# JunyiPeng00/wespeaker_hubert

Hardware: AMD Instinct MI355X
Metric: embeddings/sec on 5s 16kHz utts (higher is better)
Workload: dtype f32 (bf16x3 split MFMA, fp32 accumulate)

## Files before the change

### wespeaker_hubert_amd/csrc/conv_gemm.hip

```cpp
#include "gemm_common.h"

namespace wsp {

namespace {

constexpr int BK = 32;
constexpr int LDK = BK + 4;

template <int WM, int WN, int TM, int TN, int AMODE, bool UNI>
__global__ __launch_bounds__(256, 2) void conv_gemm_f32(const ConvGemmArgs p) {
  constexpr int BM = WM * TM * 32;
  constexpr int BN = WN * TN * 32;
  constexpr int AR = BM / 32;
  constexpr int BR = BN / 32;
  static_assert(WM * WN == 4, "4 waves");

  extern __shared__ __attribute__((aligned(16))) float smem[];
  float* As = smem;
  float* Bs = smem + 2 * BM * LDK;

  const int tid = threadIdx.x;
  const int lane = tid & 63;
  const int wave = tid >> 6;
  const int ntiles = p.N / BN;
// ... 89 lines not shown

template <int WM, int WN, int TM, int TN>
void launch_tile(const ConvGemmArgs& p, hipStream_t s) {
  const bool uni = uniform_ktiles(p);
  if (p.amode == kAAdd) {
    if (uni) launch_k<WM, WN, TM, TN, kAAdd, true>(p, s);
    else launch_k<WM, WN, TM, TN, kAAdd, false>(p, s);
  } else {
    if (uni) launch_k<WM, WN, TM, TN, kACat, true>(p, s);
    else launch_k<WM, WN, TM, TN, kACat, false>(p, s);
  }
}

}

int conv_gemm_tile_for(int N) { return (N % 128 == 0) ? 0 : 1; }

void launch_conv_gemm(const ConvGemmArgs& args, hipStream_t s) {
  const ConvGemmArgs p = normalized(args);
  check_conv_args(p, "conv_gemm");
  WSP_CHECK(!p.colsum, "conv_gemm: column sums are a bf16x3-kernel epilogue");
  WSP_CHECK(!p.conv2d && p.N % 64 == 0, "conv_gemm (f32): 1-D convs with N % 64 == 0 only");
  WSP_CHECK(!p.gcols || p.gcols % 64 == 0, "conv_gemm (f32): grouped columns must be a multiple of 64");
  WSP_CHECK(!p.sc2d && !p.lnmode && !p.gate,
            "conv_gemm (f32): conv3 + shortcut, the LayerNorm fold and the gated A tail run on tile family 7");
  if (conv_gemm_tile_for(p.N) == 0 && !p.gcols)
    launch_tile<2, 2, 2, 2>(p, s);
  else
    launch_tile<4, 1, 1, 2>(p, s);
}

}
```

### wespeaker_hubert_amd/csrc/conv_gemm_x3.hip

```cpp
#include "conv_gemm_x3_impl.h"

namespace wsp {

int conv_gemm_x3_block_rows(const ConvGemmArgs& p, int variant) {
  if (p.N % 64 != 0 || (p.gcols && p.gcols % 64 != 0)) return 128;
  if (p.gcols || p.N % 128 != 0) return 128;
  return variant == 3 ? 128 : 256;
}

namespace {
__global__ __launch_bounds__(256) void colsum_mean_kernel(const double* __restrict__ part, int bm, int T, int N,
                                                          float* __restrict__ out, int ldo) {
  const int b = blockIdx.y;
  const int n = blockIdx.x * 256 + threadIdx.x;
  if (n >= N) return;
  const long r0 = (long)b * T, r1 = r0 + T;
  double v = 0.0;
  for (long mt = r0 / bm; mt * bm < r1; ++mt) {
    const int slot = (mt * bm) / T == b ? 0 : 1;
    v += part[((size_t)mt * 2 + slot) * N + n];
  }
  out[(long)b * ldo + n] = (float)(v / (double)T);
}
}

void launch_colsum_mean(const double* part, int block_rows, int T, int B, int N, float* out, int ldo,
                        hipStream_t s) {
  WSP_CHECK(block_rows > 0 && T >= block_rows && B > 0 && N > 0, "colsum_mean: bad shape");
  hipLaunchKernelGGL(colsum_mean_kernel, dim3((N + 255) / 256, B), dim3(256), 0, s, part, block_rows, T, N, out,
                     ldo);
  WSP_HIP(hipGetLastError());
}

bool conv_gemm_x3_gate_ok(const ConvGemmArgs& args, int variant) {
  return variant == 7 && args.gate && x3::g256_gate_supported(normalized(args));
}

void launch_conv_gemm_x3(const ConvGemmArgs& args, const void* whi, const void* wlo, int variant,
                         hipStream_t s) {
  const ConvGemmArgs p = normalized(args);
  check_conv_args(p, "conv_gemm_x3");
  if (p.colsum) {
    const int bm = conv_gemm_x3_block_rows(p, variant);
    WSP_CHECK(!p.seg && !p.row_bias && !p.conv2d && p.T >= bm,
              "conv_gemm_x3: column sums need a uniform batch with T >= block rows and no row bias");
  }
  WSP_CHECK(p.Kp % 64 == 0, "conv_gemm_x3: packed K must be a multiple of 64");
  WSP_CHECK(variant >= 3 && variant <= 7, "conv_gemm_x3: tile family must be 3, 4, 5, 6 or 7");
  const __bf16* h = static_cast<const __bf16*>(whi);
  const __bf16* l = static_cast<const __bf16*>(wlo);
  x3::TileFn f;
  WSP_CHECK(!p.lnmode || (variant == 7 && x3::g256_supported(p)),
            "conv_gemm_x3: the LayerNorm fold runs on tile family 7 only");
  WSP_CHECK(!p.sc2d || (variant == 7 && x3::g256_supported(p)),
            "conv_gemm_x3: conv3 + shortcut runs on tile family 7 only (N % 256 == 0, 16-B aligned operands)");
  WSP_CHECK(!p.gate || (variant == 7 && x3::g256_gate_supported(p)),
            "conv_gemm_x3: the gated A tail runs on tile family 7 only (conv_gemm_x3_gate_ok)");
  if (variant == 7 && x3::g256_supported(p)) {
    x3::t_g256(p, h, l, s);
    return;
  }
  if (variant == 7) variant = 6;
  if (p.N % 64 != 0 || (p.gcols && p.gcols % 64 != 0)) {
    f = x3::t_4x1_1x1;
  } else if (p.gcols) {
    f = variant >= 5 ? x3::t_8x1_1x2_sw : x3::t_4x1_1x2;
  } else if (p.N % 128 != 0) {
    f = x3::t_4x1_1x2;
  } else if (variant == 3) {
    f = x3::t_2x2_2x2_sw;
  } else if (variant == 4) {
    f = x3::t_4x2_2x2_sw;
  } else if (p.N % 256 == 0) {
    f = variant == 6 ? x3::t_4x2_2x4_mf16 : x3::t_4x2_2x4_sw1;
// ... 8 lines not shown
```

### wespeaker_hubert_amd/csrc/conv_gemm_x3_impl.h

```cpp
#pragma once

#include <type_traits>

#include "gemm_common.h"

namespace wsp {

namespace {

typedef __bf16 bf16x8 __attribute__((ext_vector_type(8)));
typedef __bf16 bf16x4 __attribute__((ext_vector_type(4)));

constexpr int BK = 32;

template <bool SWZ, int MF = 32>
struct Lds {
  static constexpr int ROWB = SWZ ? 64 : 80;
  static constexpr int SKEW = SWZ ? 0 : 64;
  __device__ __forceinline__ static int off(int row, int byte) {
    static_assert(MF == 32 || SWZ, "16x16 fragments need the swizzled rows");
    if constexpr (SWZ && MF == 16)
      return row * 64 + ((((byte >> 4) ^ (0x1320 >> (4 * ((row >> 2) & 3)))) & 3) << 4) + (byte & 15);
    else if constexpr (SWZ) return row * 64 + ((((byte >> 4) ^ (row >> 2)) & 3) << 4) + (byte & 15);
    else return row * 80 + byte;
// ... 281 lines not shown
    if (p.res && p.role == 2)
      launch_x3_k<WM, WN, TM, TN, kACat, true, 2, false, SWZ, NSET>(p, whi, wlo, s);
    else
      launch_x3_k<WM, WN, TM, TN, kACat, true, 0, false, SWZ, NSET>(p, whi, wlo, s);
  } else {
    launch_x3_k<WM, WN, TM, TN, kACat, true, 0, false, SWZ, NSET, MF>(p, whi, wlo, s);
  }
}

}

namespace x3 {
using TileFn = void (*)(const ConvGemmArgs&, const __bf16*, const __bf16*, hipStream_t);
void t_4x1_1x1(const ConvGemmArgs&, const __bf16*, const __bf16*, hipStream_t);
void t_4x1_1x2(const ConvGemmArgs&, const __bf16*, const __bf16*, hipStream_t);
void t_8x1_1x2_sw(const ConvGemmArgs&, const __bf16*, const __bf16*, hipStream_t);
void t_2x2_2x2_sw(const ConvGemmArgs&, const __bf16*, const __bf16*, hipStream_t);
void t_4x2_2x2_sw(const ConvGemmArgs&, const __bf16*, const __bf16*, hipStream_t);
void t_4x2_2x4_sw1(const ConvGemmArgs&, const __bf16*, const __bf16*, hipStream_t);
void t_4x2_2x4_mf16(const ConvGemmArgs&, const __bf16*, const __bf16*, hipStream_t);
bool g256_supported(const ConvGemmArgs&);
bool g256_gate_supported(const ConvGemmArgs&);
void t_g256(const ConvGemmArgs&, const __bf16*, const __bf16*, hipStream_t);
}

}
```

### wespeaker_hubert_amd/csrc/conv_gemm_x3_t6.hip

```cpp
#include "conv_gemm_x3_impl.h"

namespace wsp {
namespace {

typedef __attribute__((address_space(3))) void lds_void;
constexpr int kGA = 256 * 128, kGW = 256 * 64, kGStage = kGA + 2 * kGW;

__device__ __forceinline__ int g_aslot(int r, int c) { return r * 128 + ((c ^ ((r >> 1) & 5)) << 4); }

__device__ __forceinline__ void g_dma(__amdgpu_buffer_rsrc_t r, unsigned char* lds, int voff) {
  __builtin_amdgcn_raw_ptr_buffer_load_lds(r, (lds_void*)lds, 16, voff, 0, 0, 0);
}

constexpr int kGEpiLd = 132;
constexpr int kGEpiBytes = 8 * 32 * kGEpiLd * 4;
typedef unsigned u32x4 __attribute__((ext_vector_type(4)));

constexpr int kLnMaxParts = 8;
__device__ __forceinline__ void g_ln_row(const ConvGemmArgs& p, int row, float& mu, float& rstd) {
  const float* s = p.ln_in + (size_t)row * p.ln_parts * 2;
  float m = s[0], m2 = s[1];
#pragma unroll
  for (int k = 1; k < kLnMaxParts; ++k) {
    if (k < p.ln_parts) {
      const float d = s[2 * k] - m;
      m += d * (1.f / (float)(k + 1));
      m2 += s[2 * k + 1] + d * d * (128.f * (float)k / (float)(k + 1));
    }
  }
  mu = m;
  rstd = 1.f / sqrtf(m2 / (128.f * (float)p.ln_parts) + p.ln_eps);
}

template <int R>
__device__ __forceinline__ void g_ln_pieces(float (&m)[R], float (&m2)[R]) {
  float n = 4.f;
  auto merge = [&](int i, float mo, float m2o) {
    const float d = mo - m[i];
    m[i] = 0.5f * (m[i] + mo);
    m2[i] = (m2[i] + m2o) + d * d * (0.5f * n);
  };
#define WSP_DPP(v, ctrl) __builtin_bit_cast(float, __builtin_amdgcn_mov_dpp(__builtin_bit_cast(int, v), ctrl, 0xF, 0xF, false))
#pragma unroll
  for (int i = 0; i < R; ++i) merge(i, WSP_DPP(m[i], 0xB1), WSP_DPP(m2[i], 0xB1));
  n *= 2.f;
#pragma unroll
  for (int i = 0; i < R; ++i) merge(i, WSP_DPP(m[i], 0x4E), WSP_DPP(m2[i], 0x4E));
  n *= 2.f;
#pragma unroll
  for (int i = 0; i < R; ++i) merge(i, WSP_DPP(m[i], 0x141), WSP_DPP(m2[i], 0x141));
  n *= 2.f;
#pragma unroll
  for (int i = 0; i < R; ++i) merge(i, WSP_DPP(m[i], 0x140), WSP_DPP(m2[i], 0x140));
  n *= 2.f;
#undef WSP_DPP
#define WSP_BC15(v) \
  __builtin_bit_cast(float, __builtin_amdgcn_update_dpp(0, __builtin_bit_cast(int, v), 0x142, 0xA, 0xF, false))
#pragma unroll
  for (int i = 0; i < R; ++i) merge(i, WSP_BC15(m[i]), WSP_BC15(m2[i]));
#undef WSP_BC15
}

template <int ACT, bool RB, bool RES, int LNM = 0>
__device__ __forceinline__ void g_epilogue_rows(const ConvGemmArgs& p, f32x4 (&acc)[4][8], int m0, int n0, int wm,
                                                int wn, int wave, int lane, unsigned char* smem, float lmu = 0.f,
                                                float lrs = 1.f) {
  float* stg = reinterpret_cast<float*>(smem) + wave * 32 * kGEpiLd;
  const int c16 = lane & 15, q = lane >> 4;
  const int cl = 4 * (lane & 31);
  const int col = n0 + wn * 128 + cl;
  const f32x4 bv = p.bias ? *reinterpret_cast<const f32x4*>(p.bias + col) : f32x4{0.f, 0.f, 0.f, 0.f};
  const f32x4 sc = p.scale ? *reinterpret_cast<const f32x4*>(p.scale + col) : f32x4{1.f, 1.f, 1.f, 1.f};
  const f32x4 sh = p.scale ? *reinterpret_cast<const f32x4*>(p.shift + col) : f32x4{0.f, 0.f, 0.f, 0.f};
  f32x4 lcs{0.f, 0.f, 0.f, 0.f}, lg{1.f, 1.f, 1.f, 1.f}, lb{0.f, 0.f, 0.f, 0.f};
  if constexpr ((LNM & 2) != 0) lcs = *reinterpret_cast<const f32x4*>(p.ln_cs + col);
  if constexpr ((LNM & 4) != 0) {
    lg = *reinterpret_cast<const f32x4*>(p.ln_g + col);
    lb = *reinterpret_cast<const f32x4*>(p.ln_b + col);
  }
  const int lparts = p.N / 128, lpart = (n0 + wn * 128) / 128;
  const __amdgpu_buffer_rsrc_t ro = make_rsrc(p.out);
  const __amdgpu_buffer_rsrc_t rres = make_rsrc(RES ? p.res : p.out);
#pragma unroll
  for (int h = 0; h < 2; ++h) {
    float pm[(LNM & 1) ? 16 : 1], pm2[(LNM & 1) ? 16 : 1];
#pragma unroll
    for (int i2 = 0; i2 < 2; ++i2)
#pragma unroll
      for (int j = 0; j < 8; ++j)
#pragma unroll
        for (int r = 0; r < 4; ++r) stg[(i2 * 16 + 4 * q + r) * kGEpiLd + j * 16 + c16] = acc[2 * h + i2][j][r];
    asm volatile("s_waitcnt lgkmcnt(0)" ::: "memory");
#pragma unroll
    for (int u = 0; u < 16; ++u) {
      const int rl = 2 * u + (lane >> 5);
      const int row = m0 + wm * 64 + h * 32 + rl;
      const bool ok = row < p.M;
      const f32x4 x = *reinterpret_cast<const f32x4*>(stg + rl * kGEpiLd + cl);
      f32x4 rv{0.f, 0.f, 0.f, 0.f}, rb{0.f, 0.f, 0.f, 0.f};
      if constexpr (RES) rv = bload4(rres, ok ? (row * p.ldres + col) * 4 : kOOB);
      if constexpr (RB) {
        const int rowc = ok ? row : p.M - 1;
        const int ub = p.seg ? seg_of(p.seg, p.nseg, rowc) : rowc / p.T;
        rb = *reinterpret_cast<const f32x4*>(p.row_bias + (size_t)ub * p.N + col);
      }
      float mu = 0.f, rstd = 1.f;
      if constexpr ((LNM & 6) != 0) {
        auto rd = [](float v, int l) {
          return __builtin_bit_cast(float, __builtin_amdgcn_readlane(__builtin_bit_cast(int, v), l));
        };
        mu = lane < 32 ? rd(lmu, h * 32 + 2 * u) : rd(lmu, h * 32 + 2 * u + 1);
        rstd = lane < 32 ? rd(lrs, h * 32 + 2 * u) : rd(lrs, h * 32 + 2 * u + 1);
      }
      f32x4 y;
#pragma unroll
      for (int e = 0; e < 4; ++e) {
        float v;
        if constexpr ((LNM & 2) != 0) v = (x[e] - mu * lcs[e]) * rstd + bv[e];
        else v = x[e] + bv[e];
        if constexpr ((LNM & 4) != 0) v += (rv[e] - mu) * rstd * lg[e] + lb[e];
        else if constexpr (RES) v += rv[e];
        if constexpr (RB) v += rb[e];
        if constexpr (ACT == kActRelu) v = fmaxf(v, 0.f);
        else if constexpr (ACT == kActTanh) v = tanhf(v);
        else if constexpr (ACT == kActGelu) v = gelu_as(v);
        y[e] = v * sc[e] + sh[e];
      }
      __builtin_amdgcn_raw_buffer_store_b128(__builtin_bit_cast(u32x4, y), ro, ok ? (row * p.ldo + col) * 4 : kOOB, 0,
                                             0);
      if constexpr ((LNM & 1) != 0) {
        pm[u] = ((y[0] + y[1]) + (y[2] + y[3])) * 0.25f;
        float q2 = 0.f;
#pragma unroll
        for (int e = 0; e < 4; ++e) q2 += (y[e] - pm[u]) * (y[e] - pm[u]);
        pm2[u] = q2;
      }
    }
    if constexpr ((LNM & 1) != 0) {
      g_ln_pieces<16>(pm, pm2);
      if ((lane & 31) == 16) {
#pragma unroll
        for (int u = 0; u < 16; ++u) {
          const int row = m0 + wm * 64 + h * 32 + 2 * u + (lane >> 5);
          if (row < p.M) *reinterpret_cast<float2*>(p.ln_out + ((size_t)row * lparts + lpart) * 2) = float2{pm[u], pm2[u]};
        }
      }
    }
    asm volatile("s_waitcnt lgkmcnt(0)" ::: "memory");
  }
}

constexpr int kGCsLd = 68;
constexpr int kGCsBytes = 8 * 64 * kGCsLd * 4;
template <int ACT>
__device__ __forceinline__ void g_epilogue_cs(const ConvGemmArgs& p, f32x4 (&acc)[4][8], int m0, int n0, int wm,
                                              int wn, int wave, int lane, unsigned char* smem) {
  float* stg = reinterpret_cast<float*>(smem) + wave * 64 * kGCsLd;
  const int c16 = lane & 15, q = lane >> 4;
  const int cl = 4 * c16;
  const __amdgpu_buffer_rsrc_t ro = make_rsrc(p.out);
  const int nb = min((m0 / p.T + 1) * p.T, p.M) - m0, mb = p.M - m0;
  unsigned side0 = 0, side1 = 0;
#pragma unroll
  for (int k = 0; k < 16; ++k) {
    const int rr = wm * 64 + (k >> 2) * 16 + 4 * q + (k & 3);
    side0 |= (rr < nb ? 1u : 0u) << k;
    side1 |= (rr >= nb && rr < mb ? 1u : 0u) << k;
  }
  double rs[8][2];
#pragma unroll
  for (int pp = 0; pp < 2; ++pp) {
#pragma unroll
    for (int i = 0; i < 4; ++i)
// ... 370 lines not shown
```

### wespeaker_hubert_amd/csrc/ecapa_model.cpp

```cpp
#include "astp_fused.h"
#include "model_impl.h"
#include "res2_chain.h"
#include "xi_pool.h"

namespace wsp {

namespace {
struct Ecapa final : Model::Impl {
  using Impl::Impl;
  int C = 512;
  bool glob = false;
  bool xi = false;
  ConvW layer1;
  struct Block {
    ConvW c1, c3, res2[7];
    LinW se1, se2;
    void* r2w = nullptr;
    float *r2b = nullptr, *r2s = nullptr, *r2t = nullptr;
  } blk[3];
  ConvW conv, pool1, pool2;
  ConvW conv_g;
  void* pool2_frag = nullptr;
  LinW pool1_ctx;
  float *prior_mean = nullptr, *prior_logprec = nullptr;
// ... 231 lines not shown
  ConvGemmArgs gcat{};
  gcat.amode = kACat;
  gcat.a[0] = x[2];
  gcat.a[1] = x[3];
  gcat.a[2] = x[4];
  gcat.cseg[1] = C;
  gcat.cseg[2] = 2 * C;
  gcat.cseg[3] = 3 * C;
  gcat.lda[0] = gcat.lda[1] = gcat.lda[2] = C;
  const ConvW& wcat = opt.cat_gate ? conv_g : conv;
  bool fold = false;
  if (opt.cat_gate && opt.gate_fold && opt.precision == 1) {
    ConvGemmArgs g = gcat;
    g.a[2] = h3;
    g.gate = W.gate;
    g.ldg = C;
    g.gate_k0 = 2 * C;
    fill(g, wcat, M, T, 1, 0, xp, 1536, kActRelu, nullptr, true, seg, B);
    fold = conv_gemm_x3_gate_ok(g, opt.x3_variant);
    if (fold) gcat = g;
  }

  gemm("layer1", layer1, feats, feat_dim, x[1], C, M, T, 1, 2, kActRelu, s, seg, B);
  for (int li = 0; li < 3; ++li) {
    const Block& b = blk[li];
    const int dil = li + 2;
    const float* xin = x[li + 1];
    gemm("conv1x1_CxC", b.c1, xin, C, h1, C, M, T, 1, 0, kActRelu, s, seg, B, nullptr, true, 1);
    if (opt.precision == 1 && opt.res2_fused && b.r2w) {
      Res2Args r{};
      r.x = h1;
      r.out = h2;
      r.ldx = r.ldo = C;
      r.M = M;
      r.T = T;
      r.dil = dil;
      r.variant = w == 128 ? opt.res2_variant : std::min(opt.res2_variant, 3);
      r.rout = res2_chain_rout(dil, r.variant, M);
      r.seg = seg;
      r.nseg = B;
      r.w = b.r2w;
      r.bias = b.r2b;
      r.scale = b.r2s;
      r.shift = b.r2t;
      run("res2_k3", 7 * 2.0 * M * w * 3 * w, s, [&] { launch_res2_chain(r, w, s); });
    } else {
      for (int i = 0; i < 7; ++i) {
        ConvGemmArgs g{};
        g.amode = i == 0 ? kACat : kAAdd;
        if (i == 0) {
          one_operand(g, h1, C, w);
// ... 4 lines not shown
        }
        gemm3("res2_k3", g, b.res2[i], dil, dil, h2 + i * w, C);
      }
    }
    {
      ConvGemmArgs g{};
      g.amode = kACat;
      g.a[0] = h2;
      g.a[1] = h1 + 7 * w;
      g.a[2] = h1;
      g.cseg[1] = 7 * w;
      g.cseg[2] = g.cseg[3] = C;
      g.role = 1;
      if (se_fused) g.colsum = W.sesum;
      gemm3("conv1x1_CxC", g, b.c3, 1, 0, h3, C);
    }
    run("se", 0, s, [&] {
      if (se_fused) launch_colsum_mean(W.sesum, se_bm, T, B, C, W.gmean, C, s);
      else launch_frame_stats(h3, C, B, T, C, W.gmean, C, 0, 0, s, seg);
      launch_small_linear({W.gmean, C, b.se1.wt, b.se1.bias, W.ghid, 128, B, C, 128, 1}, s);
      launch_small_linear({W.ghid, 128, b.se2.wt, b.se2.bias, W.gate, C, B, 128, C, 3}, s);
    });
    if (li == 2 && fold) continue;
    run("se.scale", 0, s, [&] {
      launch_residual_scale(opt.cat_gate && li == 2 ? nullptr : xin, h3, W.gate, x[li + 2], B, T, C, s, seg, M);
    });
  }
  gemm3("conv_cat", gcat, wcat, 1, 0, xp, 1536);
  if (glob) {
    run("glob_ctx", 0, s, [&] {
      launch_frame_stats(xp, 1536, B, T, 1536, W.gstats, 3072, 1, 1536, s, seg);
      launch_small_linear({W.gstats, 3072, pool1_ctx.wt, pool1_ctx.bias, W.rowb, 128, B, 3072, 128, 0}, s);
    });
  }
  if (xi) {
    gemm("xi_lin1", pool1, xp, 1536, W.att, 256, M, T, 1, 0, kActRelu, s, seg, B);
    gemm("xi_lin2", pool2, W.att, 256, W.logit, 1536, M, T, 1, 0, kActNone, s, seg, B);
    const XiPoolArgs a{W.logit, 1536, xp, 1536, prior_mean, prior_logprec, B, T, 1536, seg, W.pooled, 1536};
    run("xi_pool", 0, s, [&] { launch_xi_pool(a, s); });
    run("head", 0, s, [&] {
      launch_small_linear({W.pooled, 1536, head.wt, head.bias, embed, embed_dim, B, 1536, embed_dim, 0}, s);
    });
    return;
  }
  gemm("pool_linear1", pool1, xp, 1536, W.att, 128, M, T, 1, 0, kActTanh, s, seg, B, glob ? W.rowb : nullptr, !glob);
  if (opt.precision == 1 && opt.astp_fused) {
// ... 13 lines not shown
```

### wespeaker_hubert_amd/csrc/kernels.h

```cpp
#pragma once

#include <vector>

#include "common.h"

namespace wsp {

enum AMode { kACat = 0, kAAdd = 1 };
enum Act { kActNone = 0, kActRelu = 1, kActTanh = 2, kActGelu = 3 };

struct ConvGemmArgs {
  const float* a[3];
  int lda[3];
  int cseg[4];
  int cin, taps, dil, pad;
  int M, T, N;
  const float* w;
  int K, Kp;
  const float* bias;
  const float* row_bias;
  const float* res;
  int ldres;
  const float* scale;
  const float* shift;
  float* out;
  int ldo;
  int act;
  int amode;
  int role;
  int conv2d;
  int Fi, Ti, Fo, To, stride, kw;
  int sc2d;
  int gcols, gcin;
  const int* seg;
  const int* iseg;
  int nseg;
  double* colsum;
  int lnmode;
  float* ln_out;
  const float* ln_in;
  int ln_parts;
  const float* ln_cs;
  const float* ln_g;
  const float* ln_b;
  float ln_eps;
  const float* gate;
  int ldg, gate_k0;
};

inline ConvGemmArgs normalized(ConvGemmArgs p) {
  if (!p.conv2d && !p.sc2d) {
    if (p.stride <= 0) p.stride = 1;
    if (p.Ti <= 0) p.Ti = p.T;
  }
  return p;
}

int conv_gemm_x3_block_rows(const ConvGemmArgs& p, int variant);
void launch_colsum_mean(const double* part, int block_rows, int T, int B, int N, float* out, int ldo,
                        hipStream_t s);
void launch_conv_gemm_x3(const ConvGemmArgs& p, const void* whi, const void* wlo, int variant,
                         hipStream_t s);
bool conv_gemm_x3_gate_ok(const ConvGemmArgs& p, int variant);


void launch_conv_gemm(const ConvGemmArgs& p, hipStream_t s);
int conv_gemm_tile_for(int N);

struct SmallLinearArgs {
  const float* in;
  int ldin;
  const float* wt;
  const float* bias;
  float* out;
  int ldo;
  int R, K, N;
  int act;
  float* scratch = nullptr;
  size_t scratch_floats = 0;
};
void launch_small_linear(const SmallLinearArgs& p, hipStream_t s);
size_t small_linear_scratch_floats(int R, int N, int K);


void launch_frame_stats(const float* x, int ldx, int B, int T, int C, float* out, int ldo,
                        int with_std, int std_off, hipStream_t s, const int* seg = nullptr);
// ... 86 lines not shown
```

### wespeaker_hubert_amd/csrc/model.cpp

```cpp
#include "model_impl.h"

namespace wsp {

int detail::chunk_for(int B, size_t bytes) {
  const int bc = std::min((int)std::max<size_t>(1, kOperandCap / bytes), B);
  const int chunks = (B + bc - 1) / bc;
  return (B + chunks - 1) / chunks;
}

void Model::Impl::add(const std::string& n, std::vector<int64_t> shape) {
  idx[n] = (int)params.size();
  params.push_back(Param{n, std::move(shape), {}, false});
}
void Model::Impl::add_bn(const std::string& p, int64_t c) {
  add(p + ".weight", {c});
  add(p + ".bias", {c});
  add(p + ".running_mean", {c});
  add(p + ".running_var", {c});
  add(p + ".num_batches_tracked", {});
}
const std::vector<float>& Model::Impl::P(const std::string& n) const {
  auto it = idx.find(n);
  WSP_CHECK(it != idx.end(), "missing parameter " + n);
  const Param& p = params[it->second];
// ... 243 lines not shown
    }
  impl->prof = on;
}

namespace {
struct Opt {
  const char* key;
  int Options::*field;
  int lo, hi, hole;
  const char* err;
};
using I = Options;
constexpr int kNoHole = -1000;
const Opt kOpts[] = {
    {"precision", &I::precision, 0, 1, kNoHole, "precision must be 0 (f32) or 1 (bf16x3)"},
    {"streams", &I::streams, 1, 8, kNoHole, "streams must be 1..8"},
    {"layer", &I::layer, -1, 12, kNoHole, "layer must be -1 (weighted sum) or 0..12"},
    {"in_planes", &I::in_planes, 32, 64, kNoHole, "in_planes must be 32 or 64"},
    {"res2_fused", &I::res2_fused, 0, 1, kNoHole, "res2_fused must be 0 or 1"},
    {"cam_fused", &I::cam_fused, 0, 1, kNoHole, "cam_fused must be 0 (separate BN-ReLU pass) or 1 (GEMM prologue)"},
    {"ib_fused", &I::ib_fused, 0, 1, kNoHole, "ib_fused must be 0 (conv1, depthwise conv, conv3) or 1 (conv1, fused tail)"},
    {"cat_gate", &I::cat_gate, 0, 1, kNoHole, "cat_gate must be 0 or 1"},
    {"gate_fold", &I::gate_fold, 0, 1, kNoHole, "gate_fold must be 0 or 1"},
    {"res_prefetch", &I::res_prefetch, 0, 1, kNoHole, "res_prefetch must be 0 or 1"},
    {"res_tail", &I::res_tail, 0, 2, kNoHole, "res_tail must be 0 (off), 1 (tail + next conv1) or 2 (tail alone)"},
    {"sc_fuse", &I::sc_fuse, 0, 3, kNoHole, "sc_fuse must be 0 .. 3 (bit 0: one GEMM, bit 1: in the tail)"},
    {"c1_stage_fuse", &I::c1_stage_fuse, 0, 1, kNoHole, "c1_stage_fuse must be 0 or 1"},
    {"astp_fused", &I::astp_fused, 0, 3, kNoHole,
     "astp_fused must be 0 (linear2 GEMM + pooling kernel) or 1 (fused)"},
    {"attn_pipe", &I::attn_pipe, 0, 1, kNoHole, "attn_pipe must be 0 or 1"},
    {"pos_conv", &I::pos_conv, 0, 1, kNoHole,
     "pos_conv must be 0 (grouped implicit GEMM) or 1 (direct grouped conv)"},
    {"ln_fold", &I::ln_fold, 0, 1, kNoHole, "ln_fold must be 0 (LayerNorm kernels) or 1 (folded into the GEMMs)"},
    {"tail_batch", &I::tail_batch, 0, 1, kNoHole,
     "tail_batch must be 0 (CNN layers 4-6 per chunk) or 1 (batch-wide)"},
    {"res2_variant", &I::res2_variant, 0, 4, 1,
     "res2_variant must be 0 (4 waves, 2 x 2), 2 (4 waves on N, 4 W k-steps in flight), 3 (8 waves) "
     "or 4 (halo-free strips, c1024 widths; else as 3)"},
    {"x3_variant", &I::x3_variant, 0, 9, kNoHole,
     "x3_variant must be 3, 4, 5, 6 (5 on 16x16x32 MFMAs) or 7 (6 staged by LDS-DMA)"},
    {"conv3x3_img", &I::conv3x3_img, 0, 3, kNoHole,
     "conv3x3_img must be 0 (off), 1 (32 / 64 channels) or 2 / 3 (also 128)"},
};
const Opt& find_opt(const std::string& key) {
  for (const Opt& o : kOpts)
    if (key == o.key) return o;
// ... 52 lines not shown
```

### wespeaker_hubert_amd/csrc/model_impl.h

```cpp
#pragma once

#include <hip/hip_runtime.h>

#include <cmath>
#include <cstdint>
#include <algorithm>
#include <map>
#include <string>
#include <vector>

#include "kernels.h"
#include "model.h"
#include "pack.h"

namespace wsp {

namespace detail {

constexpr double kBnEps = 1e-5;

struct DevBuf {
  std::vector<void*> ptrs;
  ~DevBuf() {
    for (void* p : ptrs) (void)hipFree(p);
// ... 52 lines not shown
  std::vector<float> host;
  bool set = false;
  int64_t numel() const {
    int64_t n = 1;
    for (auto s : shape) n *= s;
    return n;
  }
};

struct ProfEntry {
  std::vector<std::pair<hipEvent_t, hipEvent_t>> ev;
  size_t used = 0;
  double flops = 0;
};

struct Options {
  int precision = 1;
  int x3_variant = 5;
  int streams = 1;
  int res2_fused = 1;
  int res2_variant = 4;
  int cat_gate = 1;
  int gate_fold = 1;
  int astp_fused = 1;
  int in_planes = 32;
  int conv3x3_img = 2;
  int res_prefetch = 1;
  int res_tail = 1;
  int sc_fuse = 3;
  int c1_stage_fuse = 1;
  int layer = -1;
  int attn_pipe = 1;
  int pos_conv = 1;
  int ln_fold = 0;
  int tail_batch = 1;
  int cam_fused = 1;
  int ib_fused = 0;
};

struct Model::Impl {
  std::string arch;
  int feat_dim = 80, embed_dim = 192;
  bool emb_bn = false, two_emb = false;
  Options opt;
  std::vector<Param> params;
  std::map<std::string, int> idx;
// ... 81 lines not shown
```

Measured before the change: 25730.

## Fuse SE residual scaling into next block's conv1x1 GEMM A-load (seam kernel)

Adds a seam GEMM kernel that builds the next block's conv1x1 input on the fly, as residual plus h3 times the SE gate, while loading A tiles. It writes the scaled residual out as a side product and feeds it into the bf16x3 MFMA GEMM. This removes the separate residual_scale kernel launch and one round trip of the activation through memory between ECAPA blocks. The cost is a new specialized kernel with extra A-side arithmetic and stores in its main loop, enabled by default when shape and alignment checks pass.

```diff
diff --git a/wespeaker_hubert_amd/csrc/conv_gemm.hip b/wespeaker_hubert_amd/csrc/conv_gemm.hip
--- a/wespeaker_hubert_amd/csrc/conv_gemm.hip
+++ b/wespeaker_hubert_amd/csrc/conv_gemm.hip
@@ -135,8 +135,8 @@
   WSP_CHECK(!p.colsum, "conv_gemm: column sums are a bf16x3-kernel epilogue");
   WSP_CHECK(!p.conv2d && p.N % 64 == 0, "conv_gemm (f32): 1-D convs with N % 64 == 0 only");
   WSP_CHECK(!p.gcols || p.gcols % 64 == 0, "conv_gemm (f32): grouped columns must be a multiple of 64");
-  WSP_CHECK(!p.sc2d && !p.lnmode && !p.gate,
-            "conv_gemm (f32): conv3 + shortcut, the LayerNorm fold and the gated A tail run on tile family 7");
+  WSP_CHECK(!p.sc2d && !p.lnmode && !p.gate && !p.seam_h && !p.seam_out,
+            "conv_gemm (f32): conv3 + shortcut, the LayerNorm fold, the gated A tail and the seam run on tile family 7");
   if (conv_gemm_tile_for(p.N) == 0 && !p.gcols)
     launch_tile<2, 2, 2, 2>(p, s);
   else
diff --git a/wespeaker_hubert_amd/csrc/conv_gemm_x3.hip b/wespeaker_hubert_amd/csrc/conv_gemm_x3.hip
--- a/wespeaker_hubert_amd/csrc/conv_gemm_x3.hip
+++ b/wespeaker_hubert_amd/csrc/conv_gemm_x3.hip
@@ -36,6 +36,10 @@
   return variant == 7 && args.gate && x3::g256_gate_supported(normalized(args));
 }
 
+bool conv_gemm_x3_seam_ok(const ConvGemmArgs& args, int variant) {
+  return variant == 7 && args.seam_h && x3::seam_supported(normalized(args));
+}
+
 void launch_conv_gemm_x3(const ConvGemmArgs& args, const void* whi, const void* wlo, int variant,
                          hipStream_t s) {
   const ConvGemmArgs p = normalized(args);
@@ -50,6 +54,12 @@
   const __bf16* h = static_cast<const __bf16*>(whi);
   const __bf16* l = static_cast<const __bf16*>(wlo);
   x3::TileFn f;
+  if (p.seam_h || p.seam_out) {
+    WSP_CHECK(variant == 7 && x3::seam_supported(p),
+              "conv_gemm_x3: the seam runs on tile family 7 only (conv_gemm_x3_seam_ok)");
+    x3::t_seam(p, h, l, s);
+    return;
+  }
   WSP_CHECK(!p.lnmode || (variant == 7 && x3::g256_supported(p)),
             "conv_gemm_x3: the LayerNorm fold runs on tile family 7 only");
   WSP_CHECK(!p.sc2d || (variant == 7 && x3::g256_supported(p)),
diff --git a/wespeaker_hubert_amd/csrc/conv_gemm_x3_g.h b/wespeaker_hubert_amd/csrc/conv_gemm_x3_g.h
--- /dev/null
+++ b/wespeaker_hubert_amd/csrc/conv_gemm_x3_g.h
@@ -0,0 +1,156 @@
+#pragma once
+
+#include "conv_gemm_x3_impl.h"
+
+namespace wsp {
+namespace {
+
+typedef __attribute__((address_space(3))) void lds_void;
+constexpr int kGA = 256 * 128, kGW = 256 * 64, kGStage = kGA + 2 * kGW;
+
+__device__ __forceinline__ int g_aslot(int r, int c) { return r * 128 + ((c ^ ((r >> 1) & 5)) << 4); }
+
+__device__ __forceinline__ void g_dma(__amdgpu_buffer_rsrc_t r, unsigned char* lds, int voff) {
+  __builtin_amdgcn_raw_ptr_buffer_load_lds(r, (lds_void*)lds, 16, voff, 0, 0, 0);
+}
+
+constexpr int kGEpiLd = 132;
+constexpr int kGEpiBytes = 8 * 32 * kGEpiLd * 4;
+typedef unsigned u32x4 __attribute__((ext_vector_type(4)));
+
+constexpr int kLnMaxParts = 8;
+__device__ __forceinline__ void g_ln_row(const ConvGemmArgs& p, int row, float& mu, float& rstd) {
+  const float* s = p.ln_in + (size_t)row * p.ln_parts * 2;
+  float m = s[0], m2 = s[1];
+#pragma unroll
+  for (int k = 1; k < kLnMaxParts; ++k) {
+    if (k < p.ln_parts) {
+      const float d = s[2 * k] - m;
+      m += d * (1.f / (float)(k + 1));
+      m2 += s[2 * k + 1] + d * d * (128.f * (float)k / (float)(k + 1));
+    }
+  }
+  mu = m;
+  rstd = 1.f / sqrtf(m2 / (128.f * (float)p.ln_parts) + p.ln_eps);
+}
+
+template <int R>
+__device__ __forceinline__ void g_ln_pieces(float (&m)[R], float (&m2)[R]) {
+  float n = 4.f;
+  auto merge = [&](int i, float mo, float m2o) {
+    const float d = mo - m[i];
+    m[i] = 0.5f * (m[i] + mo);
+    m2[i] = (m2[i] + m2o) + d * d * (0.5f * n);
+  };
+#define WSP_DPP(v, ctrl) __builtin_bit_cast(float, __builtin_amdgcn_mov_dpp(__builtin_bit_cast(int, v), ctrl, 0xF, 0xF, false))
+#pragma unroll
+  for (int i = 0; i < R; ++i) merge(i, WSP_DPP(m[i], 0xB1), WSP_DPP(m2[i], 0xB1));
+  n *= 2.f;
+#pragma unroll
+  for (int i = 0; i < R; ++i) merge(i, WSP_DPP(m[i], 0x4E), WSP_DPP(m2[i], 0x4E));
+  n *= 2.f;
+#pragma unroll
+  for (int i = 0; i < R; ++i) merge(i, WSP_DPP(m[i], 0x141), WSP_DPP(m2[i], 0x141));
+  n *= 2.f;
+#pragma unroll
+  for (int i = 0; i < R; ++i) merge(i, WSP_DPP(m[i], 0x140), WSP_DPP(m2[i], 0x140));
+  n *= 2.f;
+#undef WSP_DPP
+#define WSP_BC15(v) \
+  __builtin_bit_cast(float, __builtin_amdgcn_update_dpp(0, __builtin_bit_cast(int, v), 0x142, 0xA, 0xF, false))
+#pragma unroll
+  for (int i = 0; i < R; ++i) merge(i, WSP_BC15(m[i]), WSP_BC15(m2[i]));
+#undef WSP_BC15
+}
+
+template <int ACT, bool RB, bool RES, int LNM = 0>
+__device__ __forceinline__ void g_epilogue_rows(const ConvGemmArgs& p, f32x4 (&acc)[4][8], int m0, int n0, int wm,
+                                                int wn, int wave, int lane, unsigned char* smem, float lmu = 0.f,
+                                                float lrs = 1.f) {
+  float* stg = reinterpret_cast<float*>(smem) + wave * 32 * kGEpiLd;
+  const int c16 = lane & 15, q = lane >> 4;
+  const int cl = 4 * (lane & 31);
+  const int col = n0 + wn * 128 + cl;
+  const f32x4 bv = p.bias ? *reinterpret_cast<const f32x4*>(p.bias + col) : f32x4{0.f, 0.f, 0.f, 0.f};
+  const f32x4 sc = p.scale ? *reinterpret_cast<const f32x4*>(p.scale + col) : f32x4{1.f, 1.f, 1.f, 1.f};
+  const f32x4 sh = p.scale ? *reinterpret_cast<const f32x4*>(p.shift + col) : f32x4{0.f, 0.f, 0.f, 0.f};
+  f32x4 lcs{0.f, 0.f, 0.f, 0.f}, lg{1.f, 1.f, 1.f, 1.f}, lb{0.f, 0.f, 0.f, 0.f};
+  if constexpr ((LNM & 2) != 0) lcs = *reinterpret_cast<const f32x4*>(p.ln_cs + col);
+  if constexpr ((LNM & 4) != 0) {
+    lg = *reinterpret_cast<const f32x4*>(p.ln_g + col);
+    lb = *reinterpret_cast<const f32x4*>(p.ln_b + col);
+  }
+  const int lparts = p.N / 128, lpart = (n0 + wn * 128) / 128;
+  const __amdgpu_buffer_rsrc_t ro = make_rsrc(p.out);
+  const __amdgpu_buffer_rsrc_t rres = make_rsrc(RES ? p.res : p.out);
+#pragma unroll
+  for (int h = 0; h < 2; ++h) {
+    float pm[(LNM & 1) ? 16 : 1], pm2[(LNM & 1) ? 16 : 1];
+#pragma unroll
+    for (int i2 = 0; i2 < 2; ++i2)
+#pragma unroll
+      for (int j = 0; j < 8; ++j)
+#pragma unroll
+        for (int r = 0; r < 4; ++r) stg[(i2 * 16 + 4 * q + r) * kGEpiLd + j * 16 + c16] = acc[2 * h + i2][j][r];
+    asm volatile("s_waitcnt lgkmcnt(0)" ::: "memory");
+#pragma unroll
+    for (int u = 0; u < 16; ++u) {
+      const int rl = 2 * u + (lane >> 5);
+      const int row = m0 + wm * 64 + h * 32 + rl;
+      const bool ok = row < p.M;
+      const f32x4 x = *reinterpret_cast<const f32x4*>(stg + rl * kGEpiLd + cl);
+      f32x4 rv{0.f, 0.f, 0.f, 0.f}, rb{0.f, 0.f, 0.f, 0.f};
+      if constexpr (RES) rv = bload4(rres, ok ? (row * p.ldres + col) * 4 : kOOB);
+      if constexpr (RB) {
+        const int rowc = ok ? row : p.M - 1;
+        const int ub = p.seg ? seg_of(p.seg, p.nseg, rowc) : rowc / p.T;
+        rb = *reinterpret_cast<const f32x4*>(p.row_bias + (size_t)ub * p.N + col);
+      }
+      float mu = 0.f, rstd = 1.f;
+      if constexpr ((LNM & 6) != 0) {
+        auto rd = [](float v, int l) {
+          return __builtin_bit_cast(float, __builtin_amdgcn_readlane(__builtin_bit_cast(int, v), l));
+        };
+        mu = lane < 32 ? rd(lmu, h * 32 + 2 * u) : rd(lmu, h * 32 + 2 * u + 1);
+        rstd = lane < 32 ? rd(lrs, h * 32 + 2 * u) : rd(lrs, h * 32 + 2 * u + 1);
+      }
+      f32x4 y;
+#pragma unroll
+      for (int e = 0; e < 4; ++e) {
+        float v;
+        if constexpr ((LNM & 2) != 0) v = (x[e] - mu * lcs[e]) * rstd + bv[e];
+        else v = x[e] + bv[e];
+        if constexpr ((LNM & 4) != 0) v += (rv[e] - mu) * rstd * lg[e] + lb[e];
+        else if constexpr (RES) v += rv[e];
+        if constexpr (RB) v += rb[e];
+        if constexpr (ACT == kActRelu) v = fmaxf(v, 0.f);
+        else if constexpr (ACT == kActTanh) v = tanhf(v);
+        else if constexpr (ACT == kActGelu) v = gelu_as(v);
+        y[e] = v * sc[e] + sh[e];
+      }
+      __builtin_amdgcn_raw_buffer_store_b128(__builtin_bit_cast(u32x4, y), ro, ok ? (row * p.ldo + col) * 4 : kOOB, 0,
+                                             0);
+      if constexpr ((LNM & 1) != 0) {
+        pm[u] = ((y[0] + y[1]) + (y[2] + y[3])) * 0.25f;
+        float q2 = 0.f;
+#pragma unroll
+        for (int e = 0; e < 4; ++e) q2 += (y[e] - pm[u]) * (y[e] - pm[u]);
+        pm2[u] = q2;
+      }
+    }
+    if constexpr ((LNM & 1) != 0) {
+      g_ln_pieces<16>(pm, pm2);
+      if ((lane & 31) == 16) {
+#pragma unroll
+        for (int u = 0; u < 16; ++u) {
+          const int row = m0 + wm * 64 + h * 32 + 2 * u + (lane >> 5);
+          if (row < p.M) *reinterpret_cast<float2*>(p.ln_out + ((size_t)row * lparts + lpart) * 2) = float2{pm[u], pm2[u]};
+        }
+      }
+    }
+    asm volatile("s_waitcnt lgkmcnt(0)" ::: "memory");
+  }
+}
+
+}
+}
diff --git a/wespeaker_hubert_amd/csrc/conv_gemm_x3_impl.h b/wespeaker_hubert_amd/csrc/conv_gemm_x3_impl.h
--- a/wespeaker_hubert_amd/csrc/conv_gemm_x3_impl.h
+++ b/wespeaker_hubert_amd/csrc/conv_gemm_x3_impl.h
@@ -327,6 +327,8 @@
 bool g256_supported(const ConvGemmArgs&);
 bool g256_gate_supported(const ConvGemmArgs&);
 void t_g256(const ConvGemmArgs&, const __bf16*, const __bf16*, hipStream_t);
-}
-
-}
+bool seam_supported(const ConvGemmArgs&);
+void t_seam(const ConvGemmArgs&, const __bf16*, const __bf16*, hipStream_t, bool balanced = true);
+}
+
+}
diff --git a/wespeaker_hubert_amd/csrc/conv_gemm_x3_t6.hip b/wespeaker_hubert_amd/csrc/conv_gemm_x3_t6.hip
--- a/wespeaker_hubert_amd/csrc/conv_gemm_x3_t6.hip
+++ b/wespeaker_hubert_amd/csrc/conv_gemm_x3_t6.hip
@@ -1,154 +1,7 @@
-#include "conv_gemm_x3_impl.h"
+#include "conv_gemm_x3_g.h"
 
 namespace wsp {
 namespace {
-
-typedef __attribute__((address_space(3))) void lds_void;
-constexpr int kGA = 256 * 128, kGW = 256 * 64, kGStage = kGA + 2 * kGW;
-
-__device__ __forceinline__ int g_aslot(int r, int c) { return r * 128 + ((c ^ ((r >> 1) & 5)) << 4); }
-
-__device__ __forceinline__ void g_dma(__amdgpu_buffer_rsrc_t r, unsigned char* lds, int voff) {
-  __builtin_amdgcn_raw_ptr_buffer_load_lds(r, (lds_void*)lds, 16, voff, 0, 0, 0);
-}
-
-constexpr int kGEpiLd = 132;
-constexpr int kGEpiBytes = 8 * 32 * kGEpiLd * 4;
-typedef unsigned u32x4 __attribute__((ext_vector_type(4)));
-
-constexpr int kLnMaxParts = 8;
-__device__ __forceinline__ void g_ln_row(const ConvGemmArgs& p, int row, float& mu, float& rstd) {
-  const float* s = p.ln_in + (size_t)row * p.ln_parts * 2;
-  float m = s[0], m2 = s[1];
-#pragma unroll
-  for (int k = 1; k < kLnMaxParts; ++k) {
-    if (k < p.ln_parts) {
-      const float d = s[2 * k] - m;
-      m += d * (1.f / (float)(k + 1));
-      m2 += s[2 * k + 1] + d * d * (128.f * (float)k / (float)(k + 1));
-    }
-  }
-  mu = m;
-  rstd = 1.f / sqrtf(m2 / (128.f * (float)p.ln_parts) + p.ln_eps);
-}
-
-template <int R>
-__device__ __forceinline__ void g_ln_pieces(float (&m)[R], float (&m2)[R]) {
-  float n = 4.f;
-  auto merge = [&](int i, float mo, float m2o) {
-    const float d = mo - m[i];
-    m[i] = 0.5f * (m[i] + mo);
-    m2[i] = (m2[i] + m2o) + d * d * (0.5f * n);
-  };
-#define WSP_DPP(v, ctrl) __builtin_bit_cast(float, __builtin_amdgcn_mov_dpp(__builtin_bit_cast(int, v), ctrl, 0xF, 0xF, false))
-#pragma unroll
-  for (int i = 0; i < R; ++i) merge(i, WSP_DPP(m[i], 0xB1), WSP_DPP(m2[i], 0xB1));
-  n *= 2.f;
-#pragma unroll
-  for (int i = 0; i < R; ++i) merge(i, WSP_DPP(m[i], 0x4E), WSP_DPP(m2[i], 0x4E));
-  n *= 2.f;
-#pragma unroll
-  for (int i = 0; i < R; ++i) merge(i, WSP_DPP(m[i], 0x141), WSP_DPP(m2[i], 0x141));
-  n *= 2.f;
-#pragma unroll
-  for (int i = 0; i < R; ++i) merge(i, WSP_DPP(m[i], 0x140), WSP_DPP(m2[i], 0x140));
-  n *= 2.f;
-#undef WSP_DPP
-#define WSP_BC15(v) \
-  __builtin_bit_cast(float, __builtin_amdgcn_update_dpp(0, __builtin_bit_cast(int, v), 0x142, 0xA, 0xF, false))
-#pragma unroll
-  for (int i = 0; i < R; ++i) merge(i, WSP_BC15(m[i]), WSP_BC15(m2[i]));
-#undef WSP_BC15
-}
-
-template <int ACT, bool RB, bool RES, int LNM = 0>
-__device__ __forceinline__ void g_epilogue_rows(const ConvGemmArgs& p, f32x4 (&acc)[4][8], int m0, int n0, int wm,
-                                                int wn, int wave, int lane, unsigned char* smem, float lmu = 0.f,
-                                                float lrs = 1.f) {
-  float* stg = reinterpret_cast<float*>(smem) + wave * 32 * kGEpiLd;
-  const int c16 = lane & 15, q = lane >> 4;
-  const int cl = 4 * (lane & 31);
-  const int col = n0 + wn * 128 + cl;
-  const f32x4 bv = p.bias ? *reinterpret_cast<const f32x4*>(p.bias + col) : f32x4{0.f, 0.f, 0.f, 0.f};
-  const f32x4 sc = p.scale ? *reinterpret_cast<const f32x4*>(p.scale + col) : f32x4{1.f, 1.f, 1.f, 1.f};
-  const f32x4 sh = p.scale ? *reinterpret_cast<const f32x4*>(p.shift + col) : f32x4{0.f, 0.f, 0.f, 0.f};
-  f32x4 lcs{0.f, 0.f, 0.f, 0.f}, lg{1.f, 1.f, 1.f, 1.f}, lb{0.f, 0.f, 0.f, 0.f};
-  if constexpr ((LNM & 2) != 0) lcs = *reinterpret_cast<const f32x4*>(p.ln_cs + col);
-  if constexpr ((LNM & 4) != 0) {
-    lg = *reinterpret_cast<const f32x4*>(p.ln_g + col);
-    lb = *reinterpret_cast<const f32x4*>(p.ln_b + col);
-  }
-  const int lparts = p.N / 128, lpart = (n0 + wn * 128) / 128;
-  const __amdgpu_buffer_rsrc_t ro = make_rsrc(p.out);
-  const __amdgpu_buffer_rsrc_t rres = make_rsrc(RES ? p.res : p.out);
-#pragma unroll
-  for (int h = 0; h < 2; ++h) {
-    float pm[(LNM & 1) ? 16 : 1], pm2[(LNM & 1) ? 16 : 1];
-#pragma unroll
-    for (int i2 = 0; i2 < 2; ++i2)
-#pragma unroll
-      for (int j = 0; j < 8; ++j)
-#pragma unroll
-        for (int r = 0; r < 4; ++r) stg[(i2 * 16 + 4 * q + r) * kGEpiLd + j * 16 + c16] = acc[2 * h + i2][j][r];
-    asm volatile("s_waitcnt lgkmcnt(0)" ::: "memory");
-#pragma unroll
-    for (int u = 0; u < 16; ++u) {
-      const int rl = 2 * u + (lane >> 5);
-      const int row = m0 + wm * 64 + h * 32 + rl;
-      const bool ok = row < p.M;
-      const f32x4 x = *reinterpret_cast<const f32x4*>(stg + rl * kGEpiLd + cl);
-      f32x4 rv{0.f, 0.f, 0.f, 0.f}, rb{0.f, 0.f, 0.f, 0.f};
-      if constexpr (RES) rv = bload4(rres, ok ? (row * p.ldres + col) * 4 : kOOB);
-      if constexpr (RB) {
-        const int rowc = ok ? row : p.M - 1;
-        const int ub = p.seg ? seg_of(p.seg, p.nseg, rowc) : rowc / p.T;
-        rb = *reinterpret_cast<const f32x4*>(p.row_bias + (size_t)ub * p.N + col);
-      }
-      float mu = 0.f, rstd = 1.f;
-      if constexpr ((LNM & 6) != 0) {
-        auto rd = [](float v, int l) {
-          return __builtin_bit_cast(float, __builtin_amdgcn_readlane(__builtin_bit_cast(int, v), l));
-        };
-        mu = lane < 32 ? rd(lmu, h * 32 + 2 * u) : rd(lmu, h * 32 + 2 * u + 1);
-        rstd = lane < 32 ? rd(lrs, h * 32 + 2 * u) : rd(lrs, h * 32 + 2 * u + 1);
-      }
-      f32x4 y;
-#pragma unroll
-      for (int e = 0; e < 4; ++e) {
-        float v;
-        if constexpr ((LNM & 2) != 0) v = (x[e] - mu * lcs[e]) * rstd + bv[e];
-        else v = x[e] + bv[e];
-        if constexpr ((LNM & 4) != 0) v += (rv[e] - mu) * rstd * lg[e] + lb[e];
-        else if constexpr (RES) v += rv[e];
-        if constexpr (RB) v += rb[e];
-        if constexpr (ACT == kActRelu) v = fmaxf(v, 0.f);
-        else if constexpr (ACT == kActTanh) v = tanhf(v);
-        else if constexpr (ACT == kActGelu) v = gelu_as(v);
-        y[e] = v * sc[e] + sh[e];
-      }
-      __builtin_amdgcn_raw_buffer_store_b128(__builtin_bit_cast(u32x4, y), ro, ok ? (row * p.ldo + col) * 4 : kOOB, 0,
-                                             0);
-      if constexpr ((LNM & 1) != 0) {
-        pm[u] = ((y[0] + y[1]) + (y[2] + y[3])) * 0.25f;
-        float q2 = 0.f;
-#pragma unroll
-        for (int e = 0; e < 4; ++e) q2 += (y[e] - pm[u]) * (y[e] - pm[u]);
-        pm2[u] = q2;
-      }
-    }
-    if constexpr ((LNM & 1) != 0) {
-      g_ln_pieces<16>(pm, pm2);
-      if ((lane & 31) == 16) {
-#pragma unroll
-        for (int u = 0; u < 16; ++u) {
-          const int row = m0 + wm * 64 + h * 32 + 2 * u + (lane >> 5);
-          if (row < p.M) *reinterpret_cast<float2*>(p.ln_out + ((size_t)row * lparts + lpart) * 2) = float2{pm[u], pm2[u]};
-        }
-      }
-    }
-    asm volatile("s_waitcnt lgkmcnt(0)" ::: "memory");
-  }
-}
 
 constexpr int kGCsLd = 68;
 constexpr int kGCsBytes = 8 * 64 * kGCsLd * 4;
diff --git a/wespeaker_hubert_amd/csrc/conv_gemm_x3_t7.hip b/wespeaker_hubert_amd/csrc/conv_gemm_x3_t7.hip
--- /dev/null
+++ b/wespeaker_hubert_amd/csrc/conv_gemm_x3_t7.hip
@@ -0,0 +1,228 @@
+#include "conv_gemm_x3_g.h"
+
+namespace wsp {
+namespace {
+
+constexpr int kSPlane = 256 * 64;
+constexpr int kSStage = 4 * kSPlane;
+
+template <bool BAL>
+__global__ __launch_bounds__(512, 1) void conv_gemm_seam(const ConvGemmArgs p, const __bf16* __restrict__ whi,
+                                                         const __bf16* __restrict__ wlo) {
+  using L = Lds<true, 16>;
+  extern __shared__ __attribute__((aligned(16))) unsigned char smem[];
+  const int tid = threadIdx.x;
+  const int lane = tid & 63;
+  const int wave = tid >> 6;
+  const int ntiles = p.N / 256;
+  const int mtiles = (p.M + 255) / 256;
+  const int wg = xcd_remap(blockIdx.x, ntiles * mtiles);
+  const int mt = wg / ntiles;
+  const int nt = wg - mt * ntiles;
+  const int m0 = mt * 256;
+  const int n0 = nt * 256;
+  const int nk = p.K / BK;
+
+  const int srow = tid >> 3, c8 = tid & 7;
+  const __amdgpu_buffer_rsrc_t rx = make_rsrc(p.a[0]);
+  const __amdgpu_buffer_rsrc_t rh = make_rsrc(p.seam_h);
+  const __amdgpu_buffer_rsrc_t rs = make_rsrc(p.seam_out);
+  const int g_nb = min((m0 / p.T + 1) * p.T, p.M) - m0;
+  int a_r[4];
+  bool a_u[4];
+#pragma unroll
+  for (int i = 0; i < 4; ++i) {
+    const int r = srow + 64 * i;
+    a_r[i] = m0 + r < p.M ? m0 + r : -1;
+    a_u[i] = r >= g_nb;
+  }
+  f32x4 vx[4], vh[4];
+  auto load_a = [&](int kt, int i0) {
+    const int kc = kt * BK + 4 * c8;
+#pragma unroll
+    for (int i = i0; i < i0 + 2; ++i) {
+      const bool ok = kt < nk && a_r[i] >= 0;
+      vx[i] = bload4(rx, ok ? (a_r[i] * p.lda[0] + kc) * 4 : kOOB);
+      vh[i] = bload4(rh, ok ? (a_r[i] * p.ld_seam_h + kc) * 4 : kOOB);
+    }
+  };
+  int woff[2];
+#pragma unroll
+  for (int i = 0; i < 2; ++i) {
+    const int row = (2 * wave + i) * 16 + (lane >> 2);
+    const int c = (lane & 3) ^ ((0x1320 >> (4 * ((row >> 2) & 3))) & 3);
+    woff[i] = ((n0 + row) * p.Kp + 8 * c) * 2;
+  }
+  const __amdgpu_buffer_rsrc_t rwh = make_rsrc(whi);
+  const __amdgpu_buffer_rsrc_t rwl = make_rsrc(wlo);
+  auto dma_w = [&](int kt, int buf) {
+    unsigned char* st = smem + buf * kSStage;
+#pragma unroll
+    for (int i = 0; i < 2; ++i) {
+      const int o = kt < nk ? woff[i] + kt * 64 : kOOB;
+      g_dma(rwh, st + 2 * kSPlane + (2 * wave + i) * 1024, o);
+      g_dma(rwl, st + 3 * kSPlane + (2 * wave + i) * 1024, o);
+    }
+  };
+  unsigned char* const gl = smem + 2 * kSStage;
+  {
+    const __amdgpu_buffer_rsrc_t rg = make_rsrc(p.gate);
+    const int b0 = m0 / p.T, nch = p.K / 4;
+    for (int q = tid; q < 2 * nch; q += 512) {
+      const int u = q >= nch ? 1 : 0;
+      const bool ok = (b0 + u) * p.T < p.M;
+      *reinterpret_cast<f32x4*>(gl + q * 16) = bload4(rg, ok ? ((b0 + u) * p.ldg + 4 * (q - u * nch)) * 4 : kOOB);
+    }
+  }
+
+  int own = BAL ? nt : 0;
+  auto store_rows = [&](int kt, int buf, int i0) {
+#pragma clang fp contract(off)
+    unsigned char* st = smem + buf * kSStage;
+    const int kc = kt * BK + 4 * c8;
+    const int kg = kt < nk ? kc : 4 * c8;
+    const f32x4 g0 = *reinterpret_cast<const f32x4*>(gl + kg * 4);
+    const f32x4 g1 = *reinterpret_cast<const f32x4*>(gl + (p.K + kg) * 4);
+    const bool mine = (BAL || nt == 0) && kt == own && kt < nk;
+    if (mine && i0 == 2) own += BAL ? ntiles : 1;
+#pragma unroll
+    for (int i = i0; i < i0 + 2; ++i) {
+      const f32x4 g = a_u[i] ? g1 : g0;
+      f32x4 v;
+      bf16x4 hi, lo;
+#pragma unroll
+      for (int e = 0; e < 4; ++e) {
+        v[e] = __builtin_fmaf(vh[i][e], g[e], vx[i][e]);
+        const __bf16 hh = (__bf16)v[e];
+        hi[e] = hh;
+        lo[e] = (__bf16)(v[e] - (float)hh);
+      }
+      __builtin_amdgcn_raw_buffer_store_b128(__builtin_bit_cast(u32x4, v), rs,
+                                             mine && a_r[i] >= 0 ? (a_r[i] * p.ld_seam_out + kc) * 4 : kOOB, 0, 0);
+      const int off = L::off(srow + 64 * i, c8 * 8);
+      *reinterpret_cast<bf16x4*>(st + off) = hi;
+      *reinterpret_cast<bf16x4*>(st + kSPlane + off) = lo;
+    }
+  };
+
+  const int wm = wave >> 1, wn = wave & 1;
+  const int r16 = lane & 15, qk = lane >> 4;
+  f32x4 acc[4][8];
+#pragma unroll
+  for (int i = 0; i < 4; ++i)
+#pragma unroll
+    for (int j = 0; j < 8; ++j) acc[i][j] = f32x4{0.f, 0.f, 0.f, 0.f};
+  bf16x8 ah[2], al[2], bh[4], bl[4];
+  auto rdA = [&](const unsigned char* st, int ih) {
+#pragma unroll
+    for (int i = 0; i < 2; ++i) {
+      const int o = L::off(wm * 64 + (ih * 2 + i) * 16 + r16, qk * 16);
+      ah[i] = *reinterpret_cast<const bf16x8*>(st + o);
+      al[i] = *reinterpret_cast<const bf16x8*>(st + kSPlane + o);
+    }
+  };
+  auto rdB = [&](const unsigned char* st, int jh) {
+#pragma unroll
+    for (int j = 0; j < 4; ++j) {
+      const int o = L::off(wn * 128 + (jh * 4 + j) * 16 + r16, qk * 16);
+      bh[j] = *reinterpret_cast<const bf16x8*>(st + 2 * kSPlane + o);
+      bl[j] = *reinterpret_cast<const bf16x8*>(st + 3 * kSPlane + o);
+    }
+  };
+  auto mm = [&](int ih, int jh) {
+#pragma unroll
+    for (int i = 0; i < 2; ++i)
+#pragma unroll
+      for (int j = 0; j < 4; ++j) {
+        f32x4& c = acc[ih * 2 + i][jh * 4 + j];
+        c = __builtin_amdgcn_mfma_f32_16x16x32_bf16(al[i], bh[j], c, 0, 0, 0);
+        c = __builtin_amdgcn_mfma_f32_16x16x32_bf16(ah[i], bl[j], c, 0, 0, 0);
+        c = __builtin_amdgcn_mfma_f32_16x16x32_bf16(ah[i], bh[j], c, 0, 0, 0);
+      }
+  };
+
+  auto interleave = [] {
+#pragma unroll
+    for (int z = 0; z < 48; ++z) {
+      __builtin_amdgcn_sched_group_barrier(0x008, 1, 0);
+      __builtin_amdgcn_sched_group_barrier(0x002, 2, 0);
+    }
+  };
+  load_a(0, 0);
+  load_a(0, 2);
+  dma_w(0, 0);
+  asm volatile("s_waitcnt vmcnt(0) lgkmcnt(0)" ::: "memory");
+  __builtin_amdgcn_s_barrier();
+  __builtin_amdgcn_sched_barrier(0);
+  store_rows(0, 0, 0);
+  store_rows(0, 0, 2);
+  load_a(1, 0);
+  load_a(1, 2);
+  asm volatile("s_waitcnt lgkmcnt(0)" ::: "memory");
+  __builtin_amdgcn_s_barrier();
+  __builtin_amdgcn_sched_barrier(0);
+  for (int kt = 0; kt < nk; ++kt) {
+    const int buf = kt & 1;
+    const unsigned char* st = smem + buf * kSStage;
+    dma_w(kt + 1, buf ^ 1);
+    __builtin_amdgcn_sched_barrier(0);
+    rdA(st, 0);
+    rdB(st, 0);
+    mm(0, 0);
+    rdB(st, 1);
+    mm(0, 1);
+    store_rows(kt + 1, buf ^ 1, 0);
+    load_a(kt + 2, 0);
+    interleave();
+    __builtin_amdgcn_sched_barrier(0);
+    rdA(st, 1);
+    mm(1, 1);
+    rdB(st, 0);
+    mm(1, 0);
+    store_rows(kt + 1, buf ^ 1, 2);
+    load_a(kt + 2, 2);
+    interleave();
+    asm volatile("s_waitcnt vmcnt(12) lgkmcnt(0)" ::: "memory");
+    __builtin_amdgcn_s_barrier();
+    __builtin_amdgcn_sched_barrier(0);
+  }
+  switch (p.act) {
+    case kActRelu: g_epilogue_rows<kActRelu, false, false>(p, acc, m0, n0, wm, wn, wave, lane, smem); break;
+    case kActTanh: g_epilogue_rows<kActTanh, false, false>(p, acc, m0, n0, wm, wn, wave, lane, smem); break;
+    case kActGelu: g_epilogue_rows<kActGelu, false, false>(p, acc, m0, n0, wm, wn, wave, lane, smem); break;
+    default: g_epilogue_rows<kActNone, false, false>(p, acc, m0, n0, wm, wn, wave, lane, smem); break;
+  }
+}
+
+}
+
+namespace x3 {
+
+bool seam_supported(const ConvGemmArgs& p) {
+  if (!p.seam_h || !p.seam_out || !p.gate || !g256_supported(p) || !uniform_ktiles(p)) return false;
+  auto a16 = [](const void* q) { return (reinterpret_cast<uintptr_t>(q) & 15) == 0; };
+  const bool dense = p.taps == 1 && p.pad == 0 && p.stride == 1 && !p.iseg && !p.seg && p.Ti == p.T && p.cseg[1] == p.cin;
+  const bool plain = !p.colsum && !p.lnmode && !p.sc2d && !p.res && !p.row_bias;
+  const bool lds = p.K == p.Kp && p.K % 64 == 0 && p.K <= 4096;
+  const bool ops = a16(p.a[0]) && a16(p.seam_h) && a16(p.seam_out) && a16(p.gate) && p.gate_k0 == 0 && p.ldg >= p.K &&
+                   p.ldg % 4 == 0 && p.lda[0] >= p.K && p.ld_seam_h >= p.K && p.ld_seam_h % 4 == 0 &&
+                   p.ld_seam_out >= p.K && p.ld_seam_out % 4 == 0;
+  if (!dense || !plain || !lds || !ops || p.T < 256 || p.M % p.T != 0) return false;
+  const long long lim = kOOB;
+  return (long long)(p.M / p.T) * p.ldg * 4 < lim && (long long)p.M * p.ld_seam_h * 4 < lim &&
+         (long long)p.M * p.ld_seam_out * 4 < lim;
+}
+
+void t_seam(const ConvGemmArgs& p, const __bf16* h, const __bf16* l, hipStream_t s, bool balanced) {
+  WSP_CHECK(seam_supported(p), "conv_gemm_x3: the seam needs a dense 1x1 GEMM over a uniform batch with T >= 256");
+  const int nwg = ((p.M + 255) / 256) * (p.N / 256);
+  const int lds = std::max(2 * kSStage + 2 * p.K * 4, kGEpiBytes);
+  if (balanced)
+    hipLaunchKernelGGL((conv_gemm_seam<true>), dim3(nwg), dim3(512), lds, s, p, h, l);
+  else
+    hipLaunchKernelGGL((conv_gemm_seam<false>), dim3(nwg), dim3(512), lds, s, p, h, l);
+  WSP_HIP(hipGetLastError());
+}
+
+}
+}
diff --git a/wespeaker_hubert_amd/csrc/ecapa_model.cpp b/wespeaker_hubert_amd/csrc/ecapa_model.cpp
--- a/wespeaker_hubert_amd/csrc/ecapa_model.cpp
+++ b/wespeaker_hubert_amd/csrc/ecapa_model.cpp
@@ -277,11 +277,20 @@
   }
 
   gemm("layer1", layer1, feats, feat_dim, x[1], C, M, T, 1, 2, kActRelu, s, seg, B);
+  ConvGemmArgs gseam{};
+  bool seam = false;
   for (int li = 0; li < 3; ++li) {
     const Block& b = blk[li];
     const int dil = li + 2;
     const float* xin = x[li + 1];
-    gemm("conv1x1_CxC", b.c1, xin, C, h1, C, M, T, 1, 0, kActRelu, s, seg, B, nullptr, true, 1);
+    if (seam) {
+      run("se.scale", 0, s, [&] {
+        run("seam", 0, s, [&] { run("conv1x1_CxC", 2.0 * M * C * C, s, [&] { launch(gseam, b.c1, s); }); });
+      });
+      seam = false;
+    } else {
+      gemm("conv1x1_CxC", b.c1, xin, C, h1, C, M, T, 1, 0, kActRelu, s, seg, B, nullptr, true, 1);
+    }
     if (opt.precision == 1 && opt.res2_fused && b.r2w) {
       Res2Args r{};
       r.x = h1;
@@ -332,6 +341,23 @@
       launch_small_linear({W.ghid, 128, b.se2.wt, b.se2.bias, W.gate, C, B, 128, C, 3}, s);
     });
     if (li == 2 && fold) continue;
+    if (li < 2 && opt.seam_fold && opt.precision == 1) {
+      ConvGemmArgs g{};
+      one_operand(g, xin, C, C);
+      g.role = 1;
+      g.seam_h = h3;
+      g.ld_seam_h = C;
+      g.gate = W.gate;
+      g.ldg = C;
+      g.seam_out = x[li + 2];
+      g.ld_seam_out = C;
+      fill(g, blk[li + 1].c1, M, T, 1, 0, h1, C, kActRelu, nullptr, true, seg, B);
+      seam = conv_gemm_x3_seam_ok(g, opt.x3_variant);
+      if (seam) {
+        gseam = g;
+        continue;
+      }
+    }
     run("se.scale", 0, s, [&] {
       launch_residual_scale(opt.cat_gate && li == 2 ? nullptr : xin, h3, W.gate, x[li + 2], B, T, C, s, seg, M);
     });
diff --git a/wespeaker_hubert_amd/csrc/kernels.h b/wespeaker_hubert_amd/csrc/kernels.h
--- a/wespeaker_hubert_amd/csrc/kernels.h
+++ b/wespeaker_hubert_amd/csrc/kernels.h
@@ -46,6 +46,10 @@
   float ln_eps;
   const float* gate;
   int ldg, gate_k0;
+  const float* seam_h;
+  int ld_seam_h;
+  float* seam_out;
+  int ld_seam_out;
 };
 
 inline ConvGemmArgs normalized(ConvGemmArgs p) {
@@ -62,6 +66,7 @@
 void launch_conv_gemm_x3(const ConvGemmArgs& p, const void* whi, const void* wlo, int variant,
                          hipStream_t s);
 bool conv_gemm_x3_gate_ok(const ConvGemmArgs& p, int variant);
+bool conv_gemm_x3_seam_ok(const ConvGemmArgs& p, int variant);
 
 
 void launch_conv_gemm(const ConvGemmArgs& p, hipStream_t s);
diff --git a/wespeaker_hubert_amd/csrc/model.cpp b/wespeaker_hubert_amd/csrc/model.cpp
--- a/wespeaker_hubert_amd/csrc/model.cpp
+++ b/wespeaker_hubert_amd/csrc/model.cpp
@@ -289,6 +289,7 @@
     {"ib_fused", &I::ib_fused, 0, 1, kNoHole, "ib_fused must be 0 (conv1, depthwise conv, conv3) or 1 (conv1, fused tail)"},
     {"cat_gate", &I::cat_gate, 0, 1, kNoHole, "cat_gate must be 0 or 1"},
     {"gate_fold", &I::gate_fold, 0, 1, kNoHole, "gate_fold must be 0 or 1"},
+    {"seam_fold", &I::seam_fold, 0, 1, kNoHole, "seam_fold must be 0 or 1"},
     {"res_prefetch", &I::res_prefetch, 0, 1, kNoHole, "res_prefetch must be 0 or 1"},
     {"res_tail", &I::res_tail, 0, 2, kNoHole, "res_tail must be 0 (off), 1 (tail + next conv1) or 2 (tail alone)"},
     {"sc_fuse", &I::sc_fuse, 0, 3, kNoHole, "sc_fuse must be 0 .. 3 (bit 0: one GEMM, bit 1: in the tail)"},
diff --git a/wespeaker_hubert_amd/csrc/model_impl.h b/wespeaker_hubert_amd/csrc/model_impl.h
--- a/wespeaker_hubert_amd/csrc/model_impl.h
+++ b/wespeaker_hubert_amd/csrc/model_impl.h
@@ -98,6 +98,7 @@
   int res2_variant = 4;
   int cat_gate = 1;
   int gate_fold = 1;
+  int seam_fold = 1;
   int astp_fused = 1;
   int in_planes = 32;
   int conv3x3_img = 2;
```

Result: faster. 26360, median of 6 (+2.5%).
